# soytony/Point-Cloud-Preprocessing-Tools

Hardware: AMD Instinct MI355X
Metric: BEV frames/sec (131k-pt HDL-64E cloud) (higher is better)
Workload: dtype f32; 1 GPU; 1000 synthetic hdl64_sweep HDL_64E clouds per GPU (mean 135646 input pts, 133312 slots), single+multi BEV, device-resident; frames_per_gpu=1000, sub_batch=500, sensor=HDL_64E, parallelism=frames x1

## Files before the change

point-cloud-preprocessing-tools_amd/csrc/bev_cell_sums.h:

```cpp
#ifndef BEV_CELL_SUMS_H
#define BEV_CELL_SUMS_H

#include "bev_dev.h"

namespace bevk {
using namespace bevx;

constexpr int kCells = kGridCells;
constexpr int kSumQ = 4;
constexpr int kSlots = 16;
constexpr int kPartSlices = kSumWaves * kSlots;
struct SumDims {
    static constexpr int cells = (kCells + kSumQ - 1) / kSumQ;
    static constexpr int hist_stride = ((cells + 1) / 2 + 3) / 4 * 4;
    static constexpr int touch_words = (cells + 31) / 32;
    static constexpr int start_words = (cells + 3) / 4 * 4;
    static constexpr size_t fixed_words = (size_t)kSumWaves * hist_stride + start_words + (size_t)kPartSlices * 64 + 2 * (size_t)cells + touch_words +
                                          (cells + 1) / 2 + 16;
    static constexpr size_t seg_words(int T) { return (size_t)(T + 4) + (size_t)(T + 3) / 4; }
    static constexpr size_t lds_bytes(int T) { return sizeof(uint32_t) * (fixed_words + seg_words(T)); }
};
static_assert(kPartSlices * 64 <= 4096, "a part's run start (12 bits) and length (13 bits) share a word with room to spare");
size_t cell_sums_lds_bytes() { return SumDims::lds_bytes(kMaxSegs); }

__device__ __forceinline__ void cell_sums_body(uint32_t *lds, const BatchPtrs &b, const Geometry &g, const int f, int quarter, int bid )
{
    TL_BEGIN;
    using D = SumDims;
    constexpr int kCellsQ = D::cells, kHistStride = D::hist_stride, kTouchWords = D::touch_words;
    uint32_t *hist = lds;
    uint32_t *start = hist + kSumWaves * kHistStride;
    float *zbuf = reinterpret_cast<float *>(start + D::start_words);
    float *sumv = zbuf + kPartSlices * 64;
    float *cntv = sumv + kCellsQ;
    uint32_t *tbits = reinterpret_cast<uint32_t *>(cntv + kCellsQ);
    uint16_t *tlist = reinterpret_cast<uint16_t *>(tbits + kTouchWords);
    uint32_t *misc = reinterpret_cast<uint32_t *>(tlist) + (kCellsQ + 1) / 2;
    const int T = g.segs;
    uint32_t *cpre = misc + 16;
    uint8_t *rs8 = reinterpret_cast<uint8_t *>(cpre + T + 4);
    uint16_t *hist16 = reinterpret_cast<uint16_t *>(hist);

    (void)bid;
    static_assert((kSumQ & (kSumQ - 1)) == 0, "the rotation below");
#ifndef BEV_EXP_NO_QROT
    quarter = (quarter + (f >> 3)) & (kSumQ - 1);
#endif
    const int tid = threadIdx.x, lane = tid & 63, wv = __builtin_amdgcn_readfirstlane(tid >> 6);
    const uint2 *ccand = b.cand + (size_t)f * T * kSeg;
    const uint32_t *fn = b.ncand + (size_t)f * T;
    PH_DECL;
    PH();

    for (int k = tid; k < kSumWaves * kHistStride; k += kSumThreads) hist[k] = 0u;
    for (int k = tid; k < kTouchWords; k += kSumThreads) tbits[k] = 0u;
    if (tid < 16) misc[tid] = 0u;
    for (int c = tid; c < kCellsQ; c += kSumThreads) {
        sumv[c] = 0.0f;
        cntv[c] = 0.01f;
    }
    {
        uint32_t cq[4], mine = 0u;
#pragma unroll
        for (int k = 0; k < 4; ++k) {
            const int t = 4 * tid + k;
            const uint32_t w = t < T ? fn[t] : 0u;
            const uint32_t sh = 8u * (uint32_t)quarter;
            cq[k] = (w >> sh) & 0xffu;
            if (t < T) rs8[t] = (uint8_t)(((w * 0x01010100u) >> sh) & 0xffu);
            mine += cq[k];
        }
        uint32_t incl = mine;
#pragma unroll
        for (int d = 1; d < 64; d <<= 1) {
            const uint32_t v = __shfl_up(incl, d);
            if (lane >= d) incl += v;
        }
        if (lane == 63) misc[4 + wv] = incl;
        lds_barrier();
        uint32_t base = incl - mine;
        for (int w = 0; w < wv; ++w) base += misc[4 + w];
#pragma unroll
        for (int k = 0; k < 4; ++k) {
            const int t = 4 * tid + k;
            if (t <= T) cpre[t] = base;
            base += cq[k];
        }
        if (tid == kSumThreads - 1 && 4 * kSumThreads <= T) cpre[T] = base;
        if (tid < 3) cpre[T + 1 + tid] = 0xffffffffu;
        lds_barrier();
        if (tid == 0) misc[4] = misc[5] = misc[6] = misc[7] = 0u;
    }
    const int GC = (int)cpre[T];
    const int G = (GC + 63) >> 6;
    const int P = (G + kPartSlices - 1) / kPartSlices;

    uint32_t key_n[kSlots];
    float z_n[kSlots];
    int n_n[kSlots];
    auto request = [&](int p) {
        const int g0 = p * kPartSlices + wv * kSlots;
        const int gl = g0 + (lane < kSlots + 1 ? lane : kSlots);
        int lo = 0;
        if (gl < G) {
            const uint32_t x = 64u * (uint32_t)gl;
            int hi = T - 1;
            while (lo < hi) {
                const int mid = (lo + hi + 1) >> 1;
                if (cpre[mid] <= x) lo = mid; else hi = mid - 1;
            }
        } else {
            lo = T - 1;
        }
#pragma unroll
        for (int j = 0; j < kSlots; ++j) {
            const bool on = g0 + j < G;
            n_n[j] = on ? (GC - 64 * (g0 + j) < 64 ? GC - 64 * (g0 + j) : 64) : 0;
            key_n[j] = 0u;
            z_n[j] = 0.f;
            if (on) {
                const int t0 = __builtin_amdgcn_readlane(lo, j), t1 = __builtin_amdgcn_readlane(lo, j + 1);
                const uint32_t i = 64u * (uint32_t)(g0 + j) + (uint32_t)lane;
                const uint32_t c1 = cpre[t0 + 1], c2 = cpre[t0 + 2], c3 = cpre[t0 + 3];
                int t = t0 + (c1 <= i ? 1 : 0) + (c2 <= i ? 1 : 0) + (c3 <= i ? 1 : 0);
                if (t1 - t0 > 3) {
#pragma unroll 1
                    for (int u = t0 + 4; u <= t1; ++u) t += cpre[u] <= i ? 1 : 0;
                }
                t = t < T ? t : T - 1;
                const uint32_t at = (uint32_t)t * (uint32_t)kSeg + rs8[t] + (i - cpre[t]);
                const uint2 kz = *reinterpret_cast<const uint2 *>(reinterpret_cast<const char *>(ccand) + 8u * at);
                key_n[j] = kz.x;
                z_n[j] = __uint_as_float(kz.y);
            }
        }
    };
    request(0);
    lds_barrier();

    uint32_t *myhist = hist + wv * kHistStride;
    constexpr int kOriginCell = (kGridRows / 2) * kGridCols + kGridCols / 2;
    static_assert(kOriginCell == 1875, "ground_cell(0.f, 0.f)");
    constexpr uint32_t kOriginIdx = (uint32_t)kOriginCell / kSumQ;
    const bool origin_here = quarter == kOriginCell % kSumQ;
    uint32_t origin_zeros = 0u;
    bool origin_look = origin_here;
    PHA_DECL;
    for (int p = 0; p < P; ++p) {
        PHA(7);
        const int par = p & 1;
        uint32_t cell[kSlots];
        float zz[kSlots];
        int nn[kSlots];
#pragma unroll
        for (int j = 0; j < kSlots; ++j) {
            nn[j] = n_n[j];
            cell[j] = lane < nn[j] ? ((key_n[j] & kKeyCellMask) >> 2) : 0xfffu;
            zz[j] = z_n[j];
        }
#ifdef BEV_CS_TL
        asm volatile("s_waitcnt vmcnt(0)" ::: "memory");
        PHA(1);
#endif
        request(p + 1);
        if (origin_look) {
            uint32_t found = 0u;
#pragma unroll
            for (int j = 0; j < kSlots; ++j) {
                const bool zero = (cell[j] == kOriginIdx) & (zz[j] == 0.0f);
                found += zero ? 1u : 0u;
                cell[j] = zero ? 0xfffu : cell[j];
            }
            origin_zeros += found;
            origin_look = __ballot(found != 0u) != 0ull;
        }
        PHA(5);

#pragma unroll
        for (int j = 0; j < kSlots; ++j) {
            if (nn[j] == 0) break;
            const uint32_t c = cell[j];
            const bool valid = c != 0xfffu;
            const unsigned long long vb = __ballot(valid);
            uint32_t dl = 0u, dh = 0u;
#pragma unroll
            for (int bit = 0; bit < 10; ++bit) {
                int m = __builtin_amdgcn_sbfe((int)c, (uint32_t)bit, 1u);
                asm volatile("" : "+v"(m));
                const unsigned long long bal = __ballot(m != 0);
                dl = __builtin_amdgcn_bitop3_b32(dl, (uint32_t)bal, (uint32_t)m, 0xF6);
                dh = __builtin_amdgcn_bitop3_b32(dh, (uint32_t)(bal >> 32), (uint32_t)m, 0xF6);
            }
            const uint32_t pl = (uint32_t)vb & ~dl, ph = (uint32_t)(vb >> 32) & ~dh;
            const uint32_t size = (uint32_t)__popc(pl) + (uint32_t)__popc(ph);
            const uint32_t rank = __builtin_amdgcn_mbcnt_hi(ph, __builtin_amdgcn_mbcnt_lo(pl, 0u));
            const bool leader = valid && rank == 0u;
            if (leader) {
                atomicAdd(&myhist[c >> 1], size << (16 * (c & 1u)));
                atomicOr(&tbits[c >> 5], 1u << (c & 31u));
            }
            if (valid) cell[j] = c | (rank << 12) | (size << 18) | (leader ? 1u << 25 : 0u);
        }
        PHA(6);
        lds_barrier();
        if (wv == 0) {
            uint32_t word = lane < kTouchWords ? tbits[lane] : 0u;
            const uint32_t mine = (uint32_t)__popc(word);
            uint32_t incl = mine;
#pragma unroll
            for (int d = 1; d < 32; d <<= 1) {
                const uint32_t v = __shfl_up(incl, d);
                if (lane >= d) incl += v;
            }
            static_assert(kTouchWords <= 32, "one word of marks per lane of half a wave");
            if (lane == kTouchWords - 1) misc[par] = incl;
            uint32_t at = incl - mine;
            while (word) {
                const uint32_t bit = (uint32_t)__ffs((int)word) - 1u;
                word &= word - 1u;
                tlist[at++] = (uint16_t)(32u * (uint32_t)lane + bit);
            }
        }
        lds_barrier();
        PHA(0);

        const int nT = (int)misc[par];
        if (tid == 0) misc[par ^ 1] = 0u;
        for (int i0 = 0; i0 < nT; i0 += kSumThreads) {
            const int i = i0 + tid;
            uint32_t c = 0u, tot = 0u;
            if (i < nT) {
                c = tlist[i];
#pragma unroll
                for (int w = 0; w < kSumWaves; ++w) {
                    const uint32_t v = hist16[w * 2 * kHistStride + c];
                    hist16[w * 2 * kHistStride + c] = (uint16_t)tot;
                    tot += v;
                }
            }
            uint32_t incl = tot;
#pragma unroll
            for (int d = 1; d < 64; d <<= 1) {
                const uint32_t v = __shfl_up(incl, d);
                if (lane >= d) incl += v;
            }
            if (lane == 63) misc[4 + wv] = incl;
            lds_barrier();
            uint32_t run = misc[8] + incl - tot;
            for (int w = 0; w < wv; ++w) run += misc[4 + w];
            if (i < nT) start[c] = run | (tot << 16);
            lds_barrier();
            if (tid == kSumThreads - 1) misc[8] = run + tot;
        }
        lds_barrier();
        if (tid == 0) misc[8] = 0u;
        PHA(2);

#pragma unroll
        for (int j = 0; j < kSlots; ++j) {
            if (nn[j] == 0) break;
            const uint32_t v = cell[j];
            const uint32_t c = v & 0xfffu;
            if (c != 0xfffu) {
                const uint32_t off = (myhist[c >> 1] >> (16 * (c & 1u))) & 0xffffu;
                zbuf[(start[c] & 0xffffu) + off + ((v >> 12) & 63u)] = zz[j];
                if (v & (1u << 25)) atomicAdd(&myhist[c >> 1], ((v >> 18) & 127u) << (16 * (c & 1u)));
            }
        }
        lds_barrier();
        PHA(3);

        for (int k = tid; k < kTouchWords; k += kSumThreads) tbits[k] = 0u;
        for (int i = tid; i < nT; i += kSumThreads) {
            const uint32_t c = tlist[i];
            const uint32_t se = start[c];
#pragma unroll
            for (int w = 0; w < kSumWaves; ++w) hist16[w * 2 * kHistStride + c] = 0;
            int q = (int)(se & 0xffffu);
            const int e = q + (int)(se >> 16);
            float sj = sumv[c];
            cntv[c] = count_advance(cntv[c], se >> 16);
            for (; q < e && (q & 3); ++q) sj += zbuf[q];
            {
                const float4 *z4 = reinterpret_cast<const float4 *>(zbuf);
                auto add4 = [&](const float4 &v) { sj += v.x; sj += v.y; sj += v.z; sj += v.w; };
                if (q + 12 <= e) {
                    float4 a = z4[q >> 2], bq = z4[(q >> 2) + 1], cq = z4[(q >> 2) + 2];
#pragma unroll 1
                    while (q + 28 <= e) {
                        const float4 dq = z4[(q >> 2) + 3];
                        add4(a);
                        a = z4[(q >> 2) + 4];
                        add4(bq);
                        bq = z4[(q >> 2) + 5];
                        add4(cq);
                        cq = z4[(q >> 2) + 6];
                        add4(dq);
                        q += 16;
                    }
                    add4(a);
                    add4(bq);
                    add4(cq);
                    q += 12;
                }
#pragma unroll 1
                for (; q + 4 <= e; q += 4) add4(z4[q >> 2]);
            }
#pragma unroll 1
            for (; q < e; ++q) sj += zbuf[q];
            sumv[c] = sj;
        }
        lds_barrier();
        PHA(4);
    }
    if (origin_here) {
        if (tid == 0) misc[12] = 0u;
        lds_barrier();
        if (origin_zeros != 0u) atomicAdd(&misc[12], origin_zeros);
        lds_barrier();
        if (tid == 0) cntv[kOriginIdx] = count_advance(cntv[kOriginIdx], misc[12]);
        lds_barrier();
    }
    PHA_PRINT("cell_sums barrier0 - scan place sum request histloop looptop", tid == 0 && bid == 100);
    PH();
    float *avg = b.avg + (size_t)f * kCells;
    for (int c = tid; c < kCellsQ; c += kSumThreads)
        if (c * kSumQ + quarter < kCells) avg[c * kSumQ + quarter] = sumv[c] / cntv[c];
    PH_PRINT("cell_sums all-parts", tid == 0 && bid == 100);
    TL_END(K_CELL_SUMS);
#ifdef BEV_CS_TL
    if (tid == 0 && f == 12)
        printf("cell_sums frame 12 quarter %d: %d candidates, %d parts; x10 ns: list %lld scan %lld place %lld sum %lld data-wait %lld request %lld hist %lld top %lld\n",
               quarter, GC, P, pha_[0], pha_[2], pha_[3], pha_[4], pha_[1], pha_[5], pha_[6], pha_[7]);
    if (tid == 0 && bid < kWalkTlCap) {
        long long *rec = g_walk_tl[bid];
        rec[0] = ph_clk[0];
        rec[1] = wall_clock64();
        rec[2] = (long long)(unsigned)__builtin_amdgcn_s_getreg((31 << 11) | 4);
        rec[3] = (long long)(unsigned)__builtin_amdgcn_s_getreg((31 << 11) | 20) | ((long long)GC << 32) | ((long long)quarter << 8);
    }
#endif
}

__global__ __launch_bounds__(kSumThreads, 4) void k_cell_sums(BatchPtrs b, Geometry g, int nf)
{
    extern __shared__ __attribute__((aligned(16))) uint32_t lds_dyn[];
    int f, quarter;
    if (!map_block_xcd((int)blockIdx.x, nf, kSumQ, f, quarter)) return;
    cell_sums_body(lds_dyn, b, g, f, quarter, (int)blockIdx.x);
}

}

#endif
```

point-cloud-preprocessing-tools_amd/csrc/bev_resolve.h:

```cpp
#ifndef BEV_RESOLVE_H
#define BEV_RESOLVE_H

#include "bev_dev.h"

namespace bevk {
using namespace bevx;

constexpr int kResolveBatch = 4;
struct ResolveLds {
    float minavg[kGridCells];
    float avg[kGridCells];
    int edge_x[kGridRows], edge_y[kGridCols];
    uint32_t band_cursor[kMaxBands];
    uint32_t ring[kResolveThreads / 64][3][128];
    uint16_t cnt[kMaxSegs / kResolveParts + 8];
    uint8_t band_tab[512];
};
static_assert(sizeof(ResolveLds) <= 32 * 1280, "a quarter of a CU's LDS");

template <bool kPow2>
__device__ __forceinline__ void resolve_body(char *arena, const BatchPtrs &b, const Geometry &g, const int f, const int wg)
{
    TL_BEGIN;
    ResolveLds &lds_r = *reinterpret_cast<ResolveLds *>(arena);
    auto &minavg = lds_r.minavg;
    auto &avg = lds_r.avg;
    auto &edge_x = lds_r.edge_x;
    auto &edge_y = lds_r.edge_y;
    auto &band_cursor = lds_r.band_cursor;
    auto &band_tab = lds_r.band_tab;
    auto &cnt = lds_r.cnt;
    auto &ring = lds_r.ring;
    constexpr int kPartsPerWg = kResolveParts / kResolveWgs;
    const int part0 = wg * kPartsPerWg;
    const int tid = threadIdx.x, lane = tid & 63, wv = __builtin_amdgcn_readfirstlane(tid >> 6);
    const int T = g.segs;
    for (int c = tid; c < kCells; c += kResolveThreads) avg[c] = b.avg[(size_t)f * kCells + c];
    if (tid < kGridRows) edge_x[tid] = cell_edge_bin(tid, 75.0f, g.rp);
    else if (tid < kGridRows + kGridCols) edge_y[tid - kGridRows] = cell_edge_bin(tid - kGridRows, 50.0f, g.rp);
    if (tid < kMaxBands) band_cursor[tid] = 0u;
    for (int x = tid; x < g.rp.mat_size; x += kResolveThreads) band_tab[x] = (uint8_t)raster_band_of_nodiv(x, g.rp);
    lds_barrier();
    for (int c = tid; c < kCells; c += kResolveThreads) {
        const int sr = c / kGridCols, sc = c % kGridCols;
        float m = __uint_as_float(0x7fc00000u);
        if (sr - 1 >= 0) m = fminf(m, avg[c - kGridCols]);
        if (sc + 1 < kGridCols) m = fminf(m, avg[c + 1]);
        if (sc - 1 >= 0) m = fminf(m, avg[c - 1]);
        if (sr + 1 < kGridRows) m = fminf(m, avg[c + kGridCols]);
        minavg[c] = m;
    }
    lds_barrier();

    constexpr int kSl = kSeg / 64;
    constexpr int kWaves = kResolveThreads / 64;
    const int bands = g.raster_bands, lo_row = g.N - g.G, H = g.H, strips = g.strips;
    const uint2 *fcand = b.cand + (size_t)f * T * kSeg;
    const uint32_t code_cap = g.code_cap;
    const gptr<uint16_t> flabel = (gptr<uint16_t>)(b.ordered + (size_t)f * g.S);
    const bev_point_t *fordered = b.ordered + (size_t)f * g.S;
    RasterParams rp = g.rp;
    rp.max_range_f = in_vgpr(rp.max_range_f);
    rp.lidar_to_ground = in_vgpr(rp.lidar_to_ground);
    rp.mat_size = in_vgpr(rp.mat_size);
    rp.n_layers = in_vgpr(rp.n_layers);
    if (kPow2) {
        rp.inv_interval = in_vgpr(rp.inv_interval);
        rp.inv_height_res = in_vgpr(rp.inv_height_res);
    } else {
        rp.interval = in_vgpr(rp.interval);
        rp.height_res = in_vgpr(rp.height_res);
        rp.inv_interval = 0.0f;
        rp.inv_height_res = 0.0f;
    }
  for (int part = part0; part < part0 + kPartsPerWg; ++part) {
    const int t0 = (int)((long long)T * part / kResolveParts), t1 = (int)((long long)T * (part + 1) / kResolveParts);
    const gptr<uint32_t> flist = (gptr<uint32_t>)(b.code_main + ((size_t)f * g.emitters + g.strips + part) * bands * (size_t)g.code_stride);
    if (part != part0) lds_barrier();
    for (int i = tid; i < t1 - t0; i += kResolveThreads) {
        const uint32_t w = b.ncand[(size_t)f * T + t0 + i];
        cnt[i] = (uint16_t)((w & 0xffu) + ((w >> 8) & 0xffu) + ((w >> 16) & 0xffu) + (w >> 24));
    }
    if (tid < kMaxBands) band_cursor[tid] = 0u;
    lds_barrier();
    uint32_t rhead = 0u, rtail = 0u;
    auto emit = [&](uint32_t n_valid) {
        __builtin_amdgcn_wave_barrier();
        const uint32_t at = (rtail + (uint32_t)lane) & 127u;
        const uint32_t kk = ring[wv][0][at], idx = ring[wv][2][at];
        const float zz = __uint_as_float(ring[wv][1][at]);
        if ((uint32_t)lane < n_valid) {
            const int cell = (int)(kk & kKeyCellMask);
            uint32_t code;
            if (!candidate_key_escapes(kk)) {
                code = code_from_bins_t<kPow2>(edge_x[cell / kGridCols] + (int)((kk >> kKeyDxShift) & 3u),
                                               edge_y[cell % kGridCols] + (int)((kk >> kKeyDyShift) & 3u), zz, rp);
            } else {
                const float4 a = *reinterpret_cast<const float4 *>(fordered + idx);
                code = code_t<kPow2>(a.x, a.y, a.z, 1 , rp);
            }
            if (code != kSkip) {
                const int band = band_tab[code_x(code)];
                const uint32_t pos = atomicAdd(&band_cursor[band], 1u);
                flist[(uint32_t)band * g.code_stride + (pos < code_cap ? pos : code_cap - 1u)] = code;
            }
        }
        rtail += n_valid;
        __builtin_amdgcn_wave_barrier();
    };
    uint32_t key_n[kResolveBatch][kSl];
    float z_n[kResolveBatch][kSl];
    auto request = [&](int s0) {
#pragma unroll
        for (int j = 0; j < kResolveBatch; ++j) {
            const int sg = s0 + j * kWaves;
            const int n = sg < t1 ? (int)cnt[sg - t0] : 0;
#pragma unroll
            for (int k = 0; k < kSl; ++k) {
                const int last = n > 0 ? n - 1 : 0, mine = lane + 64 * k;
                const size_t at = (size_t)(sg < t1 ? sg : t0) * kSeg + (size_t)(mine < last ? mine : last);
                key_n[j][k] = 0u;
                z_n[j][k] = 0.f;
                if (64 * k < __builtin_amdgcn_readfirstlane(n)) {
                    const uint2 kz = fcand[at];
                    key_n[j][k] = kz.x;
                    z_n[j][k] = __uint_as_float(kz.y);
                }
            }
        }
    };
    request(t0 + wv);
    for (int s0 = t0 + wv; s0 < t1; s0 += kWaves * kResolveBatch) {
        uint32_t key[kResolveBatch][kSl];
        float z[kResolveBatch][kSl];
#pragma unroll
        for (int j = 0; j < kResolveBatch; ++j)
#pragma unroll
            for (int k = 0; k < kSl; ++k) {
                key[j][k] = key_n[j][k];
                z[j][k] = z_n[j][k];
            }
        if (s0 + kWaves * kResolveBatch < t1) request(s0 + kWaves * kResolveBatch);
#pragma unroll
        for (int j = 0; j < kResolveBatch; ++j) {
            const int sg = s0 + j * kWaves;
            const int n = sg < t1 ? (int)cnt[sg - t0] : 0;
            const int rr = sg / strips, strip = sg - rr * strips;
            const uint32_t slot0 = (uint32_t)((rr + lo_row - 1) * H + strip * kStripCols);
#pragma unroll
            for (int k = 0; k < kSl; ++k) {
                if (64 * k >= n) break;
                const uint32_t kk = key[j][k];
                const bool have = lane + 64 * k < n;
                const int cell = (int)(kk & kKeyCellMask);
                const bool hit = have && (z[j][k] - minavg[cell]) >= 0.3f;
                const bool pred = (kk & kKeyPredBit) != 0u;
                const bool wrong = have && hit != pred;
                const uint32_t idx = slot0 + ((kk >> kKeyColShift) & 0xffu);
                const bool coded = hit && !(kk & kKeyNoCodeBit);
                const unsigned long long cm = __ballot(coded);
                if (cm != 0ull) {
                    const uint32_t rank = __builtin_amdgcn_mbcnt_hi((uint32_t)(cm >> 32), __builtin_amdgcn_mbcnt_lo((uint32_t)cm, 0u));
                    if (coded) {
                        const uint32_t at = (rhead + rank) & 127u;
                        ring[wv][0][at] = kk;
                        ring[wv][1][at] = __float_as_uint(z[j][k]);
                        ring[wv][2][at] = idx;
                    }
                    rhead += (uint32_t)__popcll(cm);
                    if (rhead - rtail >= 64u) emit(64u);
                }
                if (wrong) {
                    flabel[16u * idx + 14u] = hit ? (uint16_t)(int16_t)-2 : (uint16_t)0;
                }
            }
        }
    }
    if (rhead != rtail) emit(rhead - rtail);
    lds_barrier();
    if (tid < bands) b.ncode[((size_t)f * g.emitters + g.strips + part) * bands + tid] = band_cursor[tid];
  }
    TL_END(K_GROUND_RESOLVE);
}

template <bool kPow2>
__global__ __launch_bounds__(kResolveThreads) void k_ground_resolve(BatchPtrs b, Geometry g)
{
    __shared__ __attribute__((aligned(16))) char arena[sizeof(ResolveLds)];
    const int f = (int)blockIdx.x / kResolveWgs;
    resolve_body<kPow2>(arena, b, g, f, (int)blockIdx.x - f * kResolveWgs);
}

}

#endif
```

Measured before the change: 420,500 frames/s.

## Prefetch per-part counts and candidate loads across parts in ground resolve

The resolve kernel now loads the per-cell averages and the segment counts for every part this workgroup owns into registers up front, and keeps one count array per part in LDS. This removes the global-load-then-barrier step at the start of each part. The first candidate batch is requested before the minavg stencil runs, and the last batch of one part prefetches the first batch of the next, so global latency overlaps compute. A small change in cell sums hoists the four ncand loads ahead of their use. The cost is more register pressure and a larger LDS footprint for the counts.

```diff
diff --git a/point-cloud-preprocessing-tools_amd/csrc/bev_cell_sums.h b/point-cloud-preprocessing-tools_amd/csrc/bev_cell_sums.h
--- a/point-cloud-preprocessing-tools_amd/csrc/bev_cell_sums.h
+++ b/point-cloud-preprocessing-tools_amd/csrc/bev_cell_sums.h
@@ -60,11 +60,13 @@
         cntv[c] = 0.01f;
     }
     {
-        uint32_t cq[4], mine = 0u;
+        uint32_t cq[4], wq[4], mine = 0u;
+#pragma unroll
+        for (int k = 0; k < 4; ++k) wq[k] = fn[4 * tid + k < T ? 4 * tid + k : T - 1];
 #pragma unroll
         for (int k = 0; k < 4; ++k) {
             const int t = 4 * tid + k;
-            const uint32_t w = t < T ? fn[t] : 0u;
+            const uint32_t w = t < T ? wq[k] : 0u;
             const uint32_t sh = 8u * (uint32_t)quarter;
             cq[k] = (w >> sh) & 0xffu;
             if (t < T) rs8[t] = (uint8_t)(((w * 0x01010100u) >> sh) & 0xffu);
diff --git a/point-cloud-preprocessing-tools_amd/csrc/bev_resolve.h b/point-cloud-preprocessing-tools_amd/csrc/bev_resolve.h
--- a/point-cloud-preprocessing-tools_amd/csrc/bev_resolve.h
+++ b/point-cloud-preprocessing-tools_amd/csrc/bev_resolve.h
@@ -13,7 +13,7 @@
     int edge_x[kGridRows], edge_y[kGridCols];
     uint32_t band_cursor[kMaxBands];
     uint32_t ring[kResolveThreads / 64][3][128];
-    uint16_t cnt[kMaxSegs / kResolveParts + 8];
+    uint16_t cnt[kResolveParts / kResolveWgs][kMaxSegs / kResolveParts + 8];
     uint8_t band_tab[512];
 };
 static_assert(sizeof(ResolveLds) <= 32 * 1280, "a quarter of a CU's LDS");
@@ -35,20 +35,40 @@
     const int part0 = wg * kPartsPerWg;
     const int tid = threadIdx.x, lane = tid & 63, wv = __builtin_amdgcn_readfirstlane(tid >> 6);
     const int T = g.segs;
-    for (int c = tid; c < kCells; c += kResolveThreads) avg[c] = b.avg[(size_t)f * kCells + c];
+    int tb[kPartsPerWg + 2];
+#pragma unroll
+    for (int pp = 0; pp < kPartsPerWg + 2; ++pp) tb[pp] = part0 + pp <= kResolveParts ? (int)((long long)T * (part0 + pp) / kResolveParts) : T;
+    auto part_t0 = [&](int part) { return tb[part - part0]; };
+    constexpr int kAvgTurns = (kCells + kResolveThreads - 1) / kResolveThreads;
+    static_assert(kMaxSegs / kResolveParts <= kResolveThreads, "one count word per thread and part");
+    const float *favg = b.avg + (size_t)f * kCells;
+    const uint32_t *fn = b.ncand + (size_t)f * T;
+    float av[kAvgTurns];
+    uint32_t cw[kPartsPerWg];
+#pragma unroll
+    for (int i = 0; i < kAvgTurns; ++i) {
+        const int c = tid + i * kResolveThreads;
+        av[i] = favg[c < kCells ? c : kCells - 1];
+    }
+#pragma unroll
+    for (int pp = 0; pp < kPartsPerWg; ++pp) {
+        const int t = part_t0(part0 + pp) + tid;
+        cw[pp] = fn[t < T ? t : T - 1];
+    }
     if (tid < kGridRows) edge_x[tid] = cell_edge_bin(tid, 75.0f, g.rp);
     else if (tid < kGridRows + kGridCols) edge_y[tid - kGridRows] = cell_edge_bin(tid - kGridRows, 50.0f, g.rp);
     if (tid < kMaxBands) band_cursor[tid] = 0u;
     for (int x = tid; x < g.rp.mat_size; x += kResolveThreads) band_tab[x] = (uint8_t)raster_band_of_nodiv(x, g.rp);
-    lds_barrier();
-    for (int c = tid; c < kCells; c += kResolveThreads) {
-        const int sr = c / kGridCols, sc = c % kGridCols;
-        float m = __uint_as_float(0x7fc00000u);
-        if (sr - 1 >= 0) m = fminf(m, avg[c - kGridCols]);
-        if (sc + 1 < kGridCols) m = fminf(m, avg[c + 1]);
-        if (sc - 1 >= 0) m = fminf(m, avg[c - 1]);
-        if (sr + 1 < kGridRows) m = fminf(m, avg[c + kGridCols]);
-        minavg[c] = m;
+#pragma unroll
+    for (int pp = 0; pp < kPartsPerWg; ++pp) {
+        const uint32_t w = cw[pp];
+        if (tid < part_t0(part0 + pp + 1) - part_t0(part0 + pp))
+            cnt[pp][tid] = (uint16_t)((w & 0xffu) + ((w >> 8) & 0xffu) + ((w >> 16) & 0xffu) + (w >> 24));
+    }
+#pragma unroll
+    for (int i = 0; i < kAvgTurns; ++i) {
+        const int c = tid + i * kResolveThreads;
+        if (c < kCells) avg[c] = av[i];
     }
     lds_barrier();
 
@@ -73,16 +93,51 @@
         rp.inv_interval = 0.0f;
         rp.inv_height_res = 0.0f;
     }
+    uint32_t key_n[kResolveBatch][kSl];
+    float z_n[kResolveBatch][kSl];
+    auto request = [&](int part, int s0) {
+        const int t0 = part_t0(part), t1 = part_t0(part + 1);
+        const uint16_t *pcnt = cnt[part - part0];
+#pragma unroll
+        for (int j = 0; j < kResolveBatch; ++j) {
+            const int sg = s0 + j * kWaves;
+            const int n = sg < t1 ? (int)pcnt[sg - t0] : 0;
+#pragma unroll
+            for (int k = 0; k < kSl; ++k) {
+                const int last = n > 0 ? n - 1 : 0, mine = lane + 64 * k;
+                const size_t at = (size_t)(sg < t1 ? sg : t0) * kSeg + (size_t)(mine < last ? mine : last);
+                key_n[j][k] = 0u;
+                z_n[j][k] = 0.f;
+                if (64 * k < __builtin_amdgcn_readfirstlane(n)) {
+                    const uint2 kz = fcand[at];
+                    key_n[j][k] = kz.x;
+                    z_n[j][k] = __uint_as_float(kz.y);
+                }
+            }
+        }
+    };
+    bool requested = part_t0(part0) + wv < part_t0(part0 + 1);
+    if (requested) request(part0, part_t0(part0) + wv);
+    for (int c = tid; c < kCells; c += kResolveThreads) {
+        const int sr = c / kGridCols, sc = c % kGridCols;
+        float m = __uint_as_float(0x7fc00000u);
+        if (sr - 1 >= 0) m = fminf(m, avg[c - kGridCols]);
+        if (sc + 1 < kGridCols) m = fminf(m, avg[c + 1]);
+        if (sc - 1 >= 0) m = fminf(m, avg[c - 1]);
+        if (sr + 1 < kGridRows) m = fminf(m, avg[c + kGridCols]);
+        minavg[c] = m;
+    }
+    lds_barrier();
+
   for (int part = part0; part < part0 + kPartsPerWg; ++part) {
-    const int t0 = (int)((long long)T * part / kResolveParts), t1 = (int)((long long)T * (part + 1) / kResolveParts);
+    const int t0 = part_t0(part), t1 = part_t0(part + 1);
+    const uint16_t *pcnt = cnt[part - part0];
     const gptr<uint32_t> flist = (gptr<uint32_t>)(b.code_main + ((size_t)f * g.emitters + g.strips + part) * bands * (size_t)g.code_stride);
-    if (part != part0) lds_barrier();
-    for (int i = tid; i < t1 - t0; i += kResolveThreads) {
-        const uint32_t w = b.ncand[(size_t)f * T + t0 + i];
-        cnt[i] = (uint16_t)((w & 0xffu) + ((w >> 8) & 0xffu) + ((w >> 16) & 0xffu) + (w >> 24));
-    }
-    if (tid < kMaxBands) band_cursor[tid] = 0u;
-    lds_barrier();
+    if (part != part0) {
+        lds_barrier();
+        if (tid < kMaxBands) band_cursor[tid] = 0u;
+        lds_barrier();
+    }
     uint32_t rhead = 0u, rtail = 0u;
     auto emit = [&](uint32_t n_valid) {
         __builtin_amdgcn_wave_barrier();
@@ -108,28 +163,8 @@
         rtail += n_valid;
         __builtin_amdgcn_wave_barrier();
     };
-    uint32_t key_n[kResolveBatch][kSl];
-    float z_n[kResolveBatch][kSl];
-    auto request = [&](int s0) {
-#pragma unroll
-        for (int j = 0; j < kResolveBatch; ++j) {
-            const int sg = s0 + j * kWaves;
-            const int n = sg < t1 ? (int)cnt[sg - t0] : 0;
-#pragma unroll
-            for (int k = 0; k < kSl; ++k) {
-                const int last = n > 0 ? n - 1 : 0, mine = lane + 64 * k;
-                const size_t at = (size_t)(sg < t1 ? sg : t0) * kSeg + (size_t)(mine < last ? mine : last);
-                key_n[j][k] = 0u;
-                z_n[j][k] = 0.f;
-                if (64 * k < __builtin_amdgcn_readfirstlane(n)) {
-                    const uint2 kz = fcand[at];
-                    key_n[j][k] = kz.x;
-                    z_n[j][k] = __uint_as_float(kz.y);
-                }
-            }
-        }
-    };
-    request(t0 + wv);
+    if (!requested && t0 + wv < t1) request(part, t0 + wv);
+    requested = false;
     for (int s0 = t0 + wv; s0 < t1; s0 += kWaves * kResolveBatch) {
         uint32_t key[kResolveBatch][kSl];
         float z[kResolveBatch][kSl];
@@ -140,11 +175,16 @@
                 key[j][k] = key_n[j][k];
                 z[j][k] = z_n[j][k];
             }
-        if (s0 + kWaves * kResolveBatch < t1) request(s0 + kWaves * kResolveBatch);
+        if (s0 + kWaves * kResolveBatch < t1) {
+            request(part, s0 + kWaves * kResolveBatch);
+        } else if (part + 1 < part0 + kPartsPerWg && t1 + wv < part_t0(part + 2)) {
+            request(part + 1, t1 + wv);
+            requested = true;
+        }
 #pragma unroll
         for (int j = 0; j < kResolveBatch; ++j) {
             const int sg = s0 + j * kWaves;
-            const int n = sg < t1 ? (int)cnt[sg - t0] : 0;
+            const int n = sg < t1 ? (int)pcnt[sg - t0] : 0;
             const int rr = sg / strips, strip = sg - rr * strips;
             const uint32_t slot0 = (uint32_t)((rr + lo_row - 1) * H + strip * kStripCols);
 #pragma unroll
```

New measurement: 423,500 frames/s, median of 2. Within noise of the previous version (+0.7%).
